# stdstu12/YUME

Measured on NVIDIA H100. Metric: latent_frames_per_sec, higher is better.
Workload: dtype bf16

## Files before the change

### yume_b200/build.py

```python
from __future__ import annotations

import hashlib
import os
import shutil
import subprocess
import sys
from pathlib import Path

ROOT = Path(__file__).resolve().parent
CSRC = ROOT / "csrc"
LIB = CSRC / "libyume_b200.so"
SOURCES = ["gemm.cu", "attention.cu", "elementwise.cu", "vae_elementwise.cu", "probe.cu", "clip.cu", "t5.cu", "gemm_fp8.cu",
           "attention_fp8.cu"]
HEADERS = ["yb_ptx.cuh", "yb_host.h", "../../include/yume_b200.h", "../../include/yume_b200_clip.h",
           "../../include/yume_b200_t5.h", "../../include/yume_b200_stream.h",
           "../../include/yume_b200_fp8.h", "../../include/yume_b200_fp8_attn.h",
           "../../include/yume_b200_fp8_vae.h"]

NVCC_FLAGS = [
    "-gencode", "arch=compute_90a,code=sm_90a",
    "-O3", "-lineinfo", "-std=c++17",
    "-Xcompiler", "-fPIC",
    "--expt-relaxed-constexpr",
    "-Xptxas", "-v",
# ... 19 lines not shown
    stamp = CSRC / ".build_stamp"
    digest = _digest()
    if not force and LIB.exists() and stamp.exists() and stamp.read_text().strip() == digest:
        return LIB
    nvcc = _nvcc()
    objs = []
    procs = []
    for src in SOURCES:
        obj = CSRC / (src[:-3] + ".o")
        cmd = [nvcc, *NVCC_FLAGS, "-c", str(CSRC / src), "-o", str(obj)]
        procs.append((src, obj, subprocess.Popen(cmd, stdout=subprocess.PIPE, stderr=subprocess.STDOUT, text=True)))
    log = []
    for src, obj, pr in procs:
        out, _ = pr.communicate()
        log.append(f"== {src}\n{out}")
        if pr.returncode != 0:
            sys.stderr.write("\n".join(log))
            raise RuntimeError(f"nvcc failed on {src}")
        objs.append(str(obj))
    tmp = LIB.with_suffix(".so.tmp")
    cmd = [nvcc, "-shared", "-gencode", "arch=compute_90a,code=sm_90a", "-o", str(tmp), *objs]
    r = subprocess.run(cmd, stdout=subprocess.PIPE, stderr=subprocess.STDOUT, text=True)
    if r.returncode != 0:
        sys.stderr.write(r.stdout)
        raise RuntimeError("nvcc link failed")
    os.replace(tmp, LIB)
    (CSRC / "build.log").write_text("\n".join(log))
    stamp.write_text(digest)
    if verbose:
        print("\n".join(log))
    return LIB


if __name__ == "__main__":
    p = build(force="--force" in sys.argv, verbose=True)
    print(f"built {p}")
```

### yume_b200/csrc/gemm.cu

```cuda
#include "yb_host.h"
#include "../../include/yume_b200_stream.h"
#include "yb_ptx.cuh"

namespace yb {

constexpr int GEMM_BLOCK_M = 128;
constexpr int GEMM_BLOCK_K = 64;
constexpr int GEMM_THREADS = 384;
constexpr int GEMM_MAX_STAGES = 8;
constexpr int GEMM_SMEM_BYTES = 227 * 1024;
constexpr int GEMM_A_BYTES = GEMM_BLOCK_M * GEMM_BLOCK_K * 2;
constexpr int GEMM_EPI_STAGE_BYTES = 8 * 16 * 36 * 4;
constexpr int GEMM_EPI_BOX_BYTES = 64 * 128;
constexpr int GEMM_EPI_TMA_BYTES = 2 * 2 * GEMM_EPI_BOX_BYTES;

struct GemmParams {
  int M, N, K;
  const float* bias;
  void* out;
  long long ldo;
  const float* gate;
  long long gate_ld;
  const int* tok_idx;
  int a_split;
  int n_split;
  long long split_stride;
  const __nv_bfloat16* res;
  long long res_ld;
  int conv, cin_chunks;
  int TW, TH, TT, tiles_w, tiles_h;
  int cT, cH, cW;
  int kh, kw;
  int off_t, off_h, off_w;
  int out_t_mul, out_t_add;
  int st_t, st_h, st_w;
  int num_m_tiles, num_n_tiles;
  int block_n, stages;
  int sk_full, sk_ns, sk_per;
  float* sk_ws;
  int tma_out;
  __nv_bfloat16* sp_peers[8];
  float* sp_sums;
  int sp_rank, sp_Lp, sp_Wh, sp_C;
};
constexpr int YB_EPI_SP_QKV = 6;

constexpr int CONVW_ROWS = GEMM_BLOCK_M + 2;
constexpr int CONVW_A_SLAB = 17 * 1024;
constexpr int CONVW_A_STAGES = 4;

__host__ __device__ constexpr int gemm_b_bytes(int block_n) { return ((block_n + 63) / 64) * 64 * GEMM_BLOCK_K * 2; }
__host__ __device__ constexpr int gemm_stage_bytes(int block_n, int convw) { return (convw ? 0 : GEMM_A_BYTES) + gemm_b_bytes(block_n); }
__host__ __device__ constexpr int gemm_a_ring_bytes(int convw) { return convw ? CONVW_A_STAGES * CONVW_A_SLAB : 0; }
__host__ __device__ constexpr bool gemm_has_tma_epilogue(int epi, int convw, int cluster) {
  return cluster == 1 && !convw && (epi == YB_EPI_BF16 || epi == YB_EPI_GELU_BF16 || epi == YB_EPI_GELU_ERF_BF16 ||
                                    epi == YB_EPI_F32 || epi == YB_EPI_GATE_RES);
}
__host__ __device__ constexpr bool gemm_tma_epilogue_only(int epi, int convw, int cluster) {
  return gemm_has_tma_epilogue(epi, convw, cluster) && epi != YB_EPI_BF16 && epi != YB_EPI_F32;
}
__host__ __device__ constexpr int gemm_epi_bytes(bool tma) { return tma ? GEMM_EPI_TMA_BYTES : GEMM_EPI_STAGE_BYTES; }
static int gemm_stages(int block_n, int convw, int epi_bytes) {
  const int s = (GEMM_SMEM_BYTES - 1024 - 256 - epi_bytes - gemm_a_ring_bytes(convw)) / gemm_stage_bytes(block_n, convw);
  return s > GEMM_MAX_STAGES ? GEMM_MAX_STAGES : s;
}

template <int EPI>
__device__ __forceinline__ void epilogue_rows16(const GemmParams& p, int col0, int my_row, int my_tok, const float* stage, int lane,
                                                float* sq) {
  constexpr bool kBf16Out = (EPI == YB_EPI_BF16 || EPI == YB_EPI_GELU_BF16 || EPI == YB_EPI_GELU_ERF_BF16 ||
                             EPI == YB_EPI_RES_BF16 || EPI == YB_EPI_SP_QKV);
  if (col0 >= p.N) return;
  if (kBf16Out) {
    const int cq = (lane & 3) * 8;
    float b[8] = {0.f, 0.f, 0.f, 0.f, 0.f, 0.f, 0.f, 0.f};
    if (p.bias) {
      const float4 b0 = __ldg(reinterpret_cast<const float4*>(p.bias + col0 + cq));
      const float4 b1 = __ldg(reinterpret_cast<const float4*>(p.bias + col0 + cq + 4));
      b[0] = b0.x; b[1] = b0.y; b[2] = b0.z; b[3] = b0.w; b[4] = b1.x; b[5] = b1.y; b[6] = b1.z; b[7] = b1.w;
    }
    long long col_off = col0 + cq;
    if (p.n_split > 0) col_off = static_cast<long long>(col0 / p.n_split) * p.split_stride + (col0 % p.n_split) + cq;
    __nv_bfloat16* obase = reinterpret_cast<__nv_bfloat16*>(p.out) + col_off;
    long long ld = p.ldo;
    if (EPI == YB_EPI_SP_QKV) {
      const int part = col0 / p.sp_C, cin = col0 - part * p.sp_C;
      const int peer = cin / p.sp_Wh;
      ld = 3LL * p.sp_Wh;
      obase = p.sp_peers[peer] + static_cast<long long>(p.sp_rank) * p.sp_Lp * ld + part * p.sp_Wh + (cin - peer * p.sp_Wh) + cq;
// ... 156 lines not shown
        if (EPI == YB_EPI_GATE_RES) tma_reduce_add_2d(tmO, buf, col0 + s * BOX_COLS, row0);
        else tma_store_2d(tmO, buf, col0 + s * BOX_COLS, row0);
        bulk_commit();
      }
      ++nbox;
    }
  }
}

template <int NM>
__device__ __forceinline__ void gemm_mma_k64(float (&acc)[128], uint32_t sa, uint32_t sb, int block_n, bool zero_first) {
  const uint64_t ad0 = make_smem_desc_sw128(sa, 16, 1024), bd0 = make_smem_desc_sw128(sb, 16, 1024);
  const int nb64 = (block_n + 63) >> 6;
#pragma unroll
  for (int k = 0; k < GEMM_BLOCK_K / 16; ++k) {
    const uint64_t ad = ad0 + 2 * k, bd = bd0 + 2 * k;
    const uint32_t accum = (zero_first && k == 0) ? 0u : 1u;
    if (NM == 256) {
      wgmma_ss_n256<0>(acc, ad, bd, accum);
    } else if (NM == 128) {
      wgmma_ss_n128<0>(acc, ad, bd, accum);
    } else {
      wgmma_ss_n64<0>(acc, ad, bd, accum);
      if (nb64 > 1) wgmma_ss_n64<32>(acc, ad, bd + (8192 >> 4), accum);
      if (nb64 > 2) wgmma_ss_n64<64>(acc, ad, bd + (16384 >> 4), accum);
      if (nb64 > 3) wgmma_ss_n64<96>(acc, ad, bd + (24576 >> 4), accum);
    }
  }
}

template <int CLUSTER>
__device__ __forceinline__ void release_slot(uint64_t* bar, int lane) {
  __syncwarp();
  if (lane == 0) {
    if (CLUSTER == 1) {
      mbar_arrive(bar);
    } else {
      mbar_arrive_cluster(bar, 0);
      mbar_arrive_cluster(bar, 1);
    }
  }
}

template <int EPI, int CONVW, int CLUSTER, int NM>
__global__ void __launch_bounds__(GEMM_THREADS, 1)
gemm_kernel(const __grid_constant__ CUtensorMap tmA, const __grid_constant__ CUtensorMap tmB, const __grid_constant__ CUtensorMap tmO,
            const GemmParams p) {
  static_assert(!(CONVW && CLUSTER != 1), "the kw-fused conv runs on single CTAs");
  constexpr bool kTmaEpi = gemm_has_tma_epilogue(EPI, CONVW, CLUSTER);
  const bool tma_out = gemm_tma_epilogue_only(EPI, CONVW, CLUSTER) || (kTmaEpi && p.tma_out);
  extern __shared__ uint8_t smem_raw[];
  uint8_t* smem = reinterpret_cast<uint8_t*>((reinterpret_cast<uintptr_t>(smem_raw) + 1023) & ~uintptr_t(1023));
  const int block_n = p.block_n, stages = p.stages;
  const int stage_bytes = gemm_stage_bytes(block_n, CONVW);
  uint8_t* a_ring = smem + stages * stage_bytes;
  float* epi = reinterpret_cast<float*>(a_ring + gemm_a_ring_bytes(CONVW));
  uint64_t* full_bar = reinterpret_cast<uint64_t*>(reinterpret_cast<uint8_t*>(epi) + gemm_epi_bytes(kTmaEpi));
  uint64_t* empty_bar = full_bar + GEMM_MAX_STAGES;
  uint64_t* a_full = empty_bar + GEMM_MAX_STAGES;
  uint64_t* a_empty = a_full + CONVW_A_STAGES;

  const int warp = threadIdx.x >> 5, lane = threadIdx.x & 31;
  const int rank = CLUSTER == 2 ? static_cast<int>(cluster_ctarank()) : 0;
  const int tile_first = blockIdx.x / CLUSTER, tile_step = gridDim.x / CLUSTER;
  const int num_tiles = p.num_m_tiles * p.num_n_tiles;
  const int num_kb = (p.K + GEMM_BLOCK_K - 1) / GEMM_BLOCK_K;
  const int num_work = p.sk_full + (num_tiles - p.sk_full) * p.sk_ns;
  auto decode_work = [&](int w, int& tile, int& kb0, int& kb1, int& part) {
    tile = w; kb0 = 0; kb1 = num_kb; part = -1;
    if (w >= p.sk_full) {
      const int u = w - p.sk_full;
      tile = p.sk_full + u / p.sk_ns;
      kb0 = (u % p.sk_ns) * p.sk_per;
      kb1 = min(num_kb, kb0 + p.sk_per);
      part = u;
    }
  };
  auto conv_box = [&](int mt, int& it, int& ih, int& iw) {
    const int per_t = p.tiles_h * p.tiles_w;
    it = mt / per_t;
    const int rem = mt - it * per_t;
    ih = rem / p.tiles_w;
    iw = rem - ih * p.tiles_w;
  };

  if (threadIdx.x == 0) {
    tma_prefetch_desc(&tmA);
    tma_prefetch_desc(&tmB);
    if (tma_out) tma_prefetch_desc(&tmO);
    for (int i = 0; i < stages; ++i) {
      mbar_init(&full_bar[i], 1);
      mbar_init(&empty_bar[i], 8 * CLUSTER);
    }
    for (int i = 0; i < (CONVW ? CONVW_A_STAGES : 0); ++i) {
      mbar_init(&a_full[i], 1);
      mbar_init(&a_empty[i], 8);
// ... 12 lines not shown
        int tile, kb0, kb1, part, m_tile, n_tile;
        decode_work(w, tile, kb0, kb1, part);
        tile_coords(tile, p.num_m_tiles, p.num_n_tiles, m_tile, n_tile);
        if (CONVW) {
          int it, ih, iw;
          conv_box(m_tile, it, ih, iw);
          const int groups = num_kb / 3;
          for (int g = 0; g < groups; ++g) {
            const int tdh = g / p.cin_chunks, cc = g - tdh * p.cin_chunks;
            const int dt = tdh / p.kh, dh = tdh - dt * p.kh;
            mbar_wait(&a_empty[a_stage], a_phase ^ 1);
            mbar_arrive_expect_tx(&a_full[a_stage], CONVW_ROWS * GEMM_BLOCK_K * 2);
            tma_load_4d(a_ring + a_stage * CONVW_A_SLAB, &tmA, &a_full[a_stage], cc * GEMM_BLOCK_K, iw * GEMM_BLOCK_M - p.off_w,
                        ih + dh - p.off_h, it + dt - p.off_t);
            if (++a_stage == CONVW_A_STAGES) {
              a_stage = 0;
              a_phase ^= 1;
            }
#pragma unroll 1
            for (int dw = 0; dw < 3; ++dw) {
              mbar_wait(&empty_bar[stage], phase ^ 1);
              mbar_arrive_expect_tx(&full_bar[stage], block_n * GEMM_BLOCK_K * 2);
              tma_load_2d(smem + stage * stage_bytes, &tmB, &full_bar[stage], ((tdh * 3 + dw) * p.cin_chunks + cc) * GEMM_BLOCK_K,
                          n_tile * block_n);
              if (++stage == stages) {
                stage = 0;
                phase ^= 1;
              }
            }
          }
          continue;
        }
        for (int kb = kb0; kb < kb1; ++kb) {
          if (CLUSTER > 1) mbar_wait_cluster(&empty_bar[stage], phase ^ 1);
          else mbar_wait(&empty_bar[stage], phase ^ 1);
          uint8_t* sa = smem + stage * stage_bytes;
          uint8_t* sb = sa + GEMM_A_BYTES;
          mbar_arrive_expect_tx(&full_bar[stage], GEMM_A_BYTES + block_n * GEMM_BLOCK_K * 2);
          const int kcol = kb * GEMM_BLOCK_K;
          const int mt = m_tile * CLUSTER + rank;
          if (p.conv) {
            const int tap = kb / p.cin_chunks, cc = kb - tap * p.cin_chunks;
            const int dt = tap / (p.kh * p.kw), dh = (tap / p.kw) % p.kh, dw = tap % p.kw;
            int it, ih, iw;
            conv_box(mt, it, ih, iw);
            tma_load_4d(sa, &tmA, &full_bar[stage], cc * GEMM_BLOCK_K, iw * p.TW * p.st_w + dw - p.off_w,
                        ih * p.TH * p.st_h + dh - p.off_h, it * p.TT * p.st_t + dt - p.off_t);
          } else {
            const int chunk = kcol / p.a_split;
            tma_load_3d(sa, &tmA, &full_bar[stage], kcol - chunk * p.a_split, mt * GEMM_BLOCK_M, chunk);
          }
          if (CLUSTER == 1) {
            tma_load_2d(sb, &tmB, &full_bar[stage], kcol, n_tile * block_n);
          } else {
            const int half = block_n / 2;
            tma_load_2d_multicast(sb + rank * half * GEMM_BLOCK_K * 2, &tmB, &full_bar[stage], kcol, n_tile * block_n + rank * half,
                                  static_cast<uint16_t>(3));
          }
          if (++stage == stages) {
            stage = 0;
            phase ^= 1;
          }
        }
      }
    }
  } else {
    setmaxnreg_inc<232>();
    const int wg = (warp >> 2) - 1;
// ... 40 lines not shown
          const uint32_t sa = smem_u32(a_ring + a_stage * CONVW_A_SLAB) + wg * 64 * 128;
#pragma unroll 1
          for (int dw = 0; dw < 3; ++dw) {
            mbar_wait(&full_bar[stage], phase);
            fence_regs(acc);
            wgmma_fence();
            gemm_mma_k64<NM>(acc, sa + dw * 128, smem_u32(smem + stage * stage_bytes), block_n, g == 0 && dw == 0);
            wgmma_commit();
            wgmma_wait<1>();
            fence_regs(acc);
            if (prev >= 0) release_slot<1>(&empty_bar[prev], lane);
            if (dw == 0 && prev_a >= 0) {
              release_slot<1>(&a_empty[prev_a], lane);
              prev_a = -1;
            }
            prev = stage;
            if (++stage == stages) {
              stage = 0;
              phase ^= 1;
            }
          }
          prev_a = a_stage;
          if (++a_stage == CONVW_A_STAGES) {
            a_stage = 0;
            a_phase ^= 1;
          }
        }
        wgmma_wait<0>();
        fence_regs(acc);
        if (prev >= 0) release_slot<1>(&empty_bar[prev], lane);
        if (prev_a >= 0) release_slot<1>(&a_empty[prev_a], lane);
      } else {
        for (int kb = kb0; kb < kb1; ++kb) {
          mbar_wait(&full_bar[stage], phase);
          const uint32_t sa = smem_u32(smem + stage * stage_bytes);
          fence_regs(acc);
          wgmma_fence();
          gemm_mma_k64<NM>(acc, sa + wg * 64 * 128, sa + GEMM_A_BYTES, block_n, kb == kb0);
          wgmma_commit();
          wgmma_wait<1>();
          fence_regs(acc);
          if (prev >= 0) release_slot<CLUSTER>(&empty_bar[prev], lane);
          prev = stage;
          if (++stage == stages) {
            stage = 0;
            phase ^= 1;
          }
        }
        wgmma_wait<0>();
        fence_regs(acc);
        if (prev >= 0) release_slot<CLUSTER>(&empty_bar[prev], lane);
      }

      const int q4 = lane >> 2, c2 = 2 * (lane & 3);
      if (part >= 0) {
        float* wbase = p.sk_ws + (static_cast<long long>(part) * 256 + rank * GEMM_BLOCK_M + r0) * block_n;
#pragma unroll
        for (int g = 0; g < 32; ++g) {
          if (g * 8 < block_n) {
            *reinterpret_cast<float2*>(wbase + q4 * block_n + g * 8 + c2) = make_float2(acc[4 * g], acc[4 * g + 1]);
            *reinterpret_cast<float2*>(wbase + (q4 + 8) * block_n + g * 8 + c2) = make_float2(acc[4 * g + 2], acc[4 * g + 3]);
          }
        }
        continue;
      }
      if (tma_out) {
        epilogue_tma<EPI, NM>(p, &tmO, acc, box_bufs, mt * GEMM_BLOCK_M + wg * 64, n_tile * block_n, wg, threadIdx.x & 127, nbox);
        continue;
      }
      int my_tok = 0;
      if (EPI == YB_EPI_GATE_RES && p.gate != nullptr && p.tok_idx != nullptr && my_row >= 0) my_tok = p.tok_idx[my_row];
      float sq[2] = {0.f, 0.f};
      auto flush_sq = [&](int part_) {
#pragma unroll
        for (int it = 0; it < 2; ++it) {
          float v = sq[it];
          v += __shfl_xor_sync(0xffffffffu, v, 1);
          v += __shfl_xor_sync(0xffffffffu, v, 2);
          const int rowi = __shfl_sync(0xffffffffu, my_row, it * 8 + (lane >> 2));
          if ((lane & 3) == 0 && rowi >= 0 && part_ < 2) atomicAdd(p.sp_sums + rowi * 2 + part_, v);
          sq[it] = 0.f;
        }
      };
      int cur_part = (EPI == YB_EPI_SP_QKV) ? (n_tile * block_n) / p.sp_C : 0;
#pragma unroll
      for (int c = 0; c < 8; ++c) {
        if (c * 32 < block_n) {
#pragma unroll
          for (int g = 0; g < 4; ++g) {
            const int i = 4 * (4 * c + g);
            *reinterpret_cast<float2*>(stage_buf + q4 * 36 + g * 8 + c2) = make_float2(acc[i], acc[i + 1]);
            *reinterpret_cast<float2*>(stage_buf + (q4 + 8) * 36 + g * 8 + c2) = make_float2(acc[i + 2], acc[i + 3]);
          }
          __syncwarp();
          const int col0 = n_tile * block_n + c * 32;
          if (EPI == YB_EPI_SP_QKV && col0 < p.N) {
            const int pt = col0 / p.sp_C;
            if (pt != cur_part) {
              flush_sq(cur_part);
              cur_part = pt;
            }
          }
          epilogue_rows16<EPI>(p, col0, my_row, my_tok, stage_buf, lane, sq);
          __syncwarp();
        }
      }
      if (EPI == YB_EPI_SP_QKV) flush_sq(cur_part);
    }
    if (tma_out && (threadIdx.x & 127) == 0) bulk_wait<0>();
  }
  if (CLUSTER > 1) cluster_sync_all();
}

__global__ void __launch_bounds__(256) gemm_splitk_combine_kernel(const GemmParams p, int tail_tiles) {
  const int block_n = p.block_n, quads = block_n >> 2;
  const long long total = static_cast<long long>(tail_tiles) * 256 * quads;
  for (long long i = blockIdx.x * static_cast<long long>(blockDim.x) + threadIdx.x; i < total;
       i += static_cast<long long>(gridDim.x) * blockDim.x) {
    const int cq = static_cast<int>(i % quads) * 4;
    const long long rr = i / quads;
    const int r = static_cast<int>(rr & 255);
    const int t = static_cast<int>(rr >> 8);
    int m_tile, n_tile;
    tile_coords(p.sk_full + t, p.num_m_tiles, p.num_n_tiles, m_tile, n_tile);
    const int row = m_tile * 256 + r, col = n_tile * block_n + cq;
    if (row >= p.M || col >= p.N) continue;
    float4 a = make_float4(0.f, 0.f, 0.f, 0.f);
    for (int sg = 0; sg < p.sk_ns; ++sg) {
      const float4 v = *reinterpret_cast<const float4*>(p.sk_ws + ((static_cast<long long>(t) * p.sk_ns + sg) * 256 + r) * block_n + cq);
      a.x += v.x; a.y += v.y; a.z += v.z; a.w += v.w;
    }
    if (p.bias) {
      const float4 b = __ldg(reinterpret_cast<const float4*>(p.bias + col));
      a.x += b.x; a.y += b.y; a.z += b.z; a.w += b.w;
    }
    float4 g = make_float4(1.f, 1.f, 1.f, 1.f);
    if (p.gate) {
      const long long tok = p.tok_idx ? p.tok_idx[row] : 0;
      g = __ldg(reinterpret_cast<const float4*>(p.gate + tok * p.gate_ld + col));
    }
    float4* xp = reinterpret_cast<float4*>(reinterpret_cast<float*>(p.out) + static_cast<long long>(row) * p.ldo + col);
    float4 x = *xp;
    x.x += a.x * g.x; x.y += a.y * g.y; x.z += a.z * g.z; x.w += a.w * g.w;
// ... 26 lines not shown
}

static int pair_block_n(int M, int N, int clusters) {
  (void)M;
  (void)clusters;
  return N >= 256 ? 256 : ((N + 31) / 32) * 32;
}

template <typename Kern>
static int pair_max_clusters(Kern kern) {
  cudaLaunchConfig_t cfg = {};
  cfg.gridDim = dim3(2 * (sm_count() / 2));
  cfg.blockDim = dim3(GEMM_THREADS);
  cfg.dynamicSmemBytes = GEMM_SMEM_BYTES;
  cudaLaunchAttribute attr;
  attr.id = cudaLaunchAttributeClusterDimension;
  attr.val.clusterDim.x = 2;
  attr.val.clusterDim.y = 1;
  attr.val.clusterDim.z = 1;
  cfg.attrs = &attr;
  cfg.numAttrs = 1;
  int n = 0;
  if (cudaOccupancyMaxActiveClusters(&n, kern, &cfg) != cudaSuccess || n <= 0) {
    (void)cudaGetLastError();
    n = sm_count() / 2;
  }
  return n;
}

template <int EPI, int CONVW, int CLUSTER>
static int launch_gemm(const CUtensorMap& tmA, const CUtensorMap& tmB, const CUtensorMap* tmO, GemmParams& p, cudaStream_t stream,
                       int split_k = 1, void* ws = nullptr, long long ws_bytes = 0) {
  static const CUtensorMap no_map = {};
  if (gemm_tma_epilogue_only(EPI, CONVW, CLUSTER) && tmO == nullptr) return YB_ERR_ARG;
  p.tma_out = gemm_has_tma_epilogue(EPI, CONVW, CLUSTER) && tmO != nullptr;
  if (!p.tma_out) tmO = &no_map;
  const int nm = p.block_n == 256 ? 2 : p.block_n == 128 ? 1 : 0;
  if (CLUSTER == 1 && nm == 0) return YB_ERR_ARG;
  auto kern = nm == 2 ? gemm_kernel<EPI, CONVW, CLUSTER, 256> : nm == 1 ? gemm_kernel<EPI, CONVW, CLUSTER, 128>
                      : gemm_kernel<EPI, CONVW, CLUSTER, CLUSTER == 1 ? 128 : 64>;
  static bool attr_set[3][kMaxDevices] = {};
  if (int rc = ensure_dynamic_smem(kern, GEMM_SMEM_BYTES, attr_set[nm], "gemm")) return rc;
  if (CLUSTER == 2) p.num_m_tiles = p.conv ? (p.num_m_tiles + 1) / 2 : (p.M + 255) / 256;
  else if (!p.conv) p.num_m_tiles = (p.M + GEMM_BLOCK_M - 1) / GEMM_BLOCK_M;
  p.num_n_tiles = (p.N + p.block_n - 1) / p.block_n;
  p.stages = gemm_stages(p.block_n, CONVW, gemm_epi_bytes(gemm_has_tma_epilogue(EPI, CONVW, CLUSTER)));
  const int tiles = p.num_m_tiles * p.num_n_tiles;
  static int max_clusters[kMaxDevices] = {0};
  const int dev = current_device();
  if (max_clusters[dev] == 0) max_clusters[dev] = CLUSTER == 2 ? pair_max_clusters(kern) : sm_count();
  p.sk_full = tiles; p.sk_ns = 1; p.sk_per = 0; p.sk_ws = nullptr;
  int tail = 0;
  if (CLUSTER == 2 && EPI == YB_EPI_GATE_RES && !p.conv && ws != nullptr && split_k != 1) {
    const int num_kb = (p.K + GEMM_BLOCK_K - 1) / GEMM_BLOCK_K;
    gemm_splitk_plan(tiles, num_kb, max_clusters[dev], split_k, &p.sk_full, &p.sk_ns, &p.sk_per);
    tail = tiles - p.sk_full;
    const long long need = static_cast<long long>(tail) * p.sk_ns * 256 * p.block_n * 4;
    if (tail > 0 && (ws_bytes < need || (reinterpret_cast<uintptr_t>(ws) & 0xF))) {
      p.sk_full = tiles; p.sk_ns = 1; tail = 0;
    }
    if (tail > 0) p.sk_ws = static_cast<float*>(ws);
  }
  const int work = p.sk_full + tail * p.sk_ns;
  const int groups = work < max_clusters[dev] ? work : max_clusters[dev];
  cudaLaunchConfig_t cfg = {};
  cfg.gridDim = dim3(groups * CLUSTER);
  cfg.blockDim = dim3(GEMM_THREADS);
  cfg.dynamicSmemBytes = GEMM_SMEM_BYTES;
  cfg.stream = stream;
  cudaLaunchAttribute attr;
  attr.id = cudaLaunchAttributeClusterDimension;
  attr.val.clusterDim.x = CLUSTER;
  attr.val.clusterDim.y = 1;
  attr.val.clusterDim.z = 1;
  cfg.attrs = &attr;
  cfg.numAttrs = 1;
  (void)cudaLaunchKernelEx(&cfg, kern, tmA, tmB, *tmO, p);
  int rc = check_launch("gemm");
  if (rc || tail == 0) return rc;
// ... 107 lines not shown
  if (a->struct_bytes != sizeof(yb_gemm_args)) return YB_ERR_ARG;
  if (a->cta_pair < 0 || a->cta_pair > 2 || a->split_k < 0 || a->split_k > 12) return YB_ERR_ARG;
  int a_split = a->K;
  long long a_chunk_ld = 0;
  if (a->a_split > 0) {
    if (a->a_split % GEMM_BLOCK_K != 0 || a->K % a->a_split != 0) return YB_ERR_SHAPE;
    a_split = a->a_split;
    a_chunk_ld = a->a_split_stride;
  }
  const int a_chunks = a->K / a_split;
  if (a->n_split < 0 || (a->n_split > 0 && (a->n_split % 32 != 0 || a->epilogue != YB_EPI_BF16))) return YB_ERR_ARG;
  GemmParams p;
  p.M = a->M;
  p.N = a->N;
  p.K = a->K;
  p.bias = static_cast<const float*>(a->bias);
  p.out = a->out;
  p.ldo = a->ldo;
  p.gate = static_cast<const float*>(a->gate);
  p.gate_ld = a->gate_ld;
  p.tok_idx = static_cast<const int*>(a->tok_idx);
  p.a_split = a_split;
  p.res = static_cast<const __nv_bfloat16*>(a->res);
  p.res_ld = a->res_ld;
  p.conv = 0;
  p.n_split = a->n_split;
  p.split_stride = a->split_stride;
  p.block_n = 0;
  p.stages = 0;
  CUtensorMap tmA, tmB;
  int rc = make_tmap_bf16_3d(&tmA, a->A, a_chunks, a->M, a_split, a->lda, a_chunks > 1 ? a_chunk_ld : a->lda * (long long)a->M + 8,
                             GEMM_BLOCK_M, GEMM_BLOCK_K);
  if (rc) return rc;
  const bool pair = a->cta_pair == 2;
  if (pair) {
    int bn = a->block_n;
    if (bn == 0) bn = pair_block_n(a->M, a->N, sm_count() / 2);
    if (bn < 32 || bn > 256 || bn % 32 != 0) return YB_ERR_ARG;
    p.block_n = bn;
    rc = make_tmap_bf16_2d(&tmB, a->B, a->N, a->K, a->ldb, bn / 2, GEMM_BLOCK_K);
    if (rc) return rc;
    switch (a->epilogue) {
      case YB_EPI_BF16: return launch_gemm<YB_EPI_BF16, 0, 2>(tmA, tmB, nullptr, p, stream);
      case YB_EPI_GELU_BF16: return launch_gemm<YB_EPI_GELU_BF16, 0, 2>(tmA, tmB, nullptr, p, stream);
      case YB_EPI_F32: return launch_gemm<YB_EPI_F32, 0, 2>(tmA, tmB, nullptr, p, stream);
      case YB_EPI_GELU_ERF_BF16: return launch_gemm<YB_EPI_GELU_ERF_BF16, 0, 2>(tmA, tmB, nullptr, p, stream);
      case YB_EPI_RES_BF16: return launch_gemm<YB_EPI_RES_BF16, 0, 2>(tmA, tmB, nullptr, p, stream);
      default: return launch_gemm<YB_EPI_GATE_RES, 0, 2>(tmA, tmB, nullptr, p, stream, a->split_k, a->ws, a->ws_bytes);
    }
  }
  const int block_n = (a->block_n == 128 || a->block_n == 256) ? a->block_n : ((a->N % 256 == 0 || a->N > 1024) ? 256 : 128);
  rc = make_tmap_bf16_2d(&tmB, a->B, a->N, a->K, a->ldb, block_n, GEMM_BLOCK_K);
  if (rc) return rc;
  p.block_n = block_n;
  CUtensorMap tmO;
  const CUtensorMap* tmo = nullptr;
  if (a->n_split == 0 && a->epilogue != YB_EPI_RES_BF16) {
    const int elem = (a->epilogue == YB_EPI_F32 || a->epilogue == YB_EPI_GATE_RES) ? 4 : 2;
    rc = make_tmap_out_2d(&tmO, a->out, a->M, a->N, a->ldo, elem, 64);
    if (rc) return rc;
    tmo = &tmO;
  }
  switch (a->epilogue) {
    case YB_EPI_BF16: return launch_gemm<YB_EPI_BF16, 0, 1>(tmA, tmB, tmo, p, stream);
    case YB_EPI_GELU_BF16: return launch_gemm<YB_EPI_GELU_BF16, 0, 1>(tmA, tmB, tmo, p, stream);
    case YB_EPI_F32: return launch_gemm<YB_EPI_F32, 0, 1>(tmA, tmB, tmo, p, stream);
    case YB_EPI_GELU_ERF_BF16: return launch_gemm<YB_EPI_GELU_ERF_BF16, 0, 1>(tmA, tmB, tmo, p, stream);
    case YB_EPI_RES_BF16: return launch_gemm<YB_EPI_RES_BF16, 0, 1>(tmA, tmB, nullptr, p, stream);
    default: return launch_gemm<YB_EPI_GATE_RES, 0, 1>(tmA, tmB, tmo, p, stream);
  }
}


static int conv3d_launch(const yb_conv3d_args* a, int t_hist, void* stream_) {
  using namespace yb;
  if (!a || !a->xpad || !a->w || !a->out) return YB_ERR_ARG;
  if (a->struct_bytes != sizeof(yb_conv3d_args)) return YB_ERR_ARG;
  if (a->T <= 0 || a->H <= 0 || a->W <= 0 || a->Cp <= 0 || a->Cout <= 0) return YB_ERR_ARG;
  if (t_hist < 0) return YB_ERR_ARG;
  if (a->Cp % 64 != 0 || a->Cout % 32 != 0) return YB_ERR_SHAPE;
  if ((a->ldo % 8) || (reinterpret_cast<uintptr_t>(a->out) & 0xF)) return YB_ERR_ALIGNMENT;
  if (a->epilogue != YB_EPI_BF16 && a->epilogue != YB_EPI_F32 && a->epilogue != YB_EPI_RES_BF16) return YB_ERR_ARG;
  if (a->epilogue == YB_EPI_RES_BF16 && (!a->res || (a->res_ld % 8))) return YB_ERR_ARG;
  cudaStream_t stream = reinterpret_cast<cudaStream_t>(stream_);
  GemmParams p;
  const int kt = a->kt > 0 ? a->kt : 3, kh = a->kh > 0 ? a->kh : 3, kw = a->kw > 0 ? a->kw : 3;
  if ((kt != 1 && kt != 3) || (kh != 1 && kh != 3) || (kw != 1 && kw != 3)) return YB_ERR_SHAPE;
  const int block_n = (a->Cout % 256 == 0) ? 256 : 128;
  bool fuse_w = false;
  if (a->cta_pair < 0 || a->cta_pair > 2) return YB_ERR_ARG;
  const int st_t = a->stride_t > 0 ? a->stride_t : 1, st_hw = a->stride_hw > 0 ? a->stride_hw : 1;
  if (st_t > 2 || st_hw > 2) return YB_ERR_ARG;
  const bool strided = st_t > 1 || st_hw > 1;
  if (strided && !a->oob_zero_pad) return YB_ERR_ARG;
  if (t_hist > 0 && (!a->oob_zero_pad || t_hist != (st_t > 1 ? 1 : kt - 1))) return YB_ERR_ARG;
// ... 41 lines not shown
    p.conv = 1;
    p.block_n = a->Cout <= 256 ? a->Cout : (a->Cout % 192 == 0 ? 192 : 256);
    CUtensorMap tmBp;
    rc = make_tmap_bf16_2d(&tmBp, a->w, a->Cout, static_cast<uint64_t>(taps) * a->Cp, static_cast<uint64_t>(taps) * a->Cp,
                           p.block_n / 2, GEMM_BLOCK_K);
    if (rc) return rc;
    switch (a->epilogue) {
      case YB_EPI_BF16: return launch_gemm<YB_EPI_BF16, 0, 2>(tmA, tmBp, nullptr, p, stream);
      case YB_EPI_F32: return launch_gemm<YB_EPI_F32, 0, 2>(tmA, tmBp, nullptr, p, stream);
      default: return launch_gemm<YB_EPI_RES_BF16, 0, 2>(tmA, tmBp, nullptr, p, stream);
    }
  }
  p.block_n = block_n;
#define YB_CONV_DISPATCH(CW)                                                                  \
  switch (a->epilogue) {                                                                     \
    case YB_EPI_BF16: return launch_gemm<YB_EPI_BF16, CW, 1>(tmA, tmB, nullptr, p, stream);   \
    case YB_EPI_F32: return launch_gemm<YB_EPI_F32, CW, 1>(tmA, tmB, nullptr, p, stream);     \
    default: return launch_gemm<YB_EPI_RES_BF16, CW, 1>(tmA, tmB, nullptr, p, stream);        \
  }
  if (fuse_w) {
    YB_CONV_DISPATCH(1)
  } else {
    YB_CONV_DISPATCH(0)
  }
#undef YB_CONV_DISPATCH
}

extern "C" int yb_conv3d_causal(const yb_conv3d_args* a, void* stream) { return conv3d_launch(a, 0, stream); }

extern "C" int yb_conv3d_causal_hist(const yb_conv3d_args* a, int t_hist, void* stream) {
  if (t_hist <= 0) return YB_ERR_ARG;
  return conv3d_launch(a, t_hist, stream);
}
```

### yume_b200/csrc/yb_ptx.cuh

```cuda
#pragma once
#include <cstdint>
#include <cstdio>
#include <cuda.h>
#include <cuda_runtime.h>
#include <cuda_bf16.h>

namespace yb {

__device__ __forceinline__ uint32_t smem_u32(const void* p) {
  return static_cast<uint32_t>(__cvta_generic_to_shared(p));
}

template <int N>
__device__ __forceinline__ void setmaxnreg_inc() {
  asm volatile("setmaxnreg.inc.sync.aligned.u32 %0;\n" ::"n"(N));
}
template <int N>
__device__ __forceinline__ void setmaxnreg_dec() {
  asm volatile("setmaxnreg.dec.sync.aligned.u32 %0;\n" ::"n"(N));
}
__device__ __forceinline__ void named_bar_sync(int id, int count) {
  asm volatile("bar.sync %0, %1;" ::"r"(id), "r"(count) : "memory");
}

// ... 35 lines not shown
      : "memory");
  return ok != 0;
}
#ifndef YB_WAIT_LIMIT_CYCLES
#define YB_WAIT_LIMIT_CYCLES 8000000000LL
#endif
__device__ __forceinline__ void mbar_wait(uint64_t* bar, uint32_t parity) {
  if (mbar_try_wait(bar, parity)) return;
  const long long t0 = clock64();
  while (!mbar_try_wait(bar, parity)) {
    if (clock64() - t0 > YB_WAIT_LIMIT_CYCLES) {
#ifdef YB_DEBUG_WAIT
      printf("yb: mbarrier wait timeout block=(%d,%d) thread=%d bar=%u parity=%u\n", blockIdx.x, blockIdx.y,
             threadIdx.x, smem_u32(bar), parity);
#endif
      __trap();
    }
  }
}
__device__ __forceinline__ void att_wait(uint64_t* bar, uint32_t parity) {
  if (mbar_try_wait(bar, parity)) return;
  const long long t0 = clock64();
  while (!mbar_try_wait(bar, parity)) {
    if (clock64() - t0 > YB_WAIT_LIMIT_CYCLES) {
#ifdef YB_DEBUG_WAIT
      printf("yb: attention consumer mbarrier wait timeout block=(%d,%d) thread=%d bar=%u parity=%u\n", blockIdx.x,
             blockIdx.y, threadIdx.x, smem_u32(bar), parity);
#endif
      asm volatile("trap;");
      break;
    }
  }
}
__device__ __forceinline__ void mbar_wait_cluster(uint64_t* bar, uint32_t parity) {
  const long long t0 = clock64();
  for (;;) {
    uint32_t ok;
    asm volatile(
        "{\n\t.reg .pred p;\n\t"
        "mbarrier.try_wait.parity.acquire.cluster.shared::cta.b64 p, [%1], %2;\n\t"
        "selp.u32 %0, 1, 0, p;\n\t}\n"
        : "=r"(ok)
        : "r"(smem_u32(bar)), "r"(parity)
        : "memory");
    if (ok) return;
    if (clock64() - t0 > YB_WAIT_LIMIT_CYCLES) __trap();
  }
}

__device__ __forceinline__ uint32_t cluster_ctarank() {
  uint32_t r;
  asm volatile("mov.u32 %0, %%cluster_ctarank;" : "=r"(r));
  return r;
}
__device__ __forceinline__ void cluster_sync_all() {
  asm volatile("barrier.cluster.arrive.release.aligned;\n\tbarrier.cluster.wait.acquire.aligned;" ::: "memory");
}
__device__ __forceinline__ void mbar_arrive_cluster(uint64_t* bar, uint32_t cta) {
  uint32_t remote;
  asm volatile("mapa.shared::cluster.u32 %0, %1, %2;" : "=r"(remote) : "r"(smem_u32(bar)), "r"(cta));
  asm volatile("mbarrier.arrive.release.cluster.shared::cluster.b64 _, [%0];" ::"r"(remote) : "memory");
}

__device__ __forceinline__ void tma_prefetch_desc(const CUtensorMap* tmap) {
  asm volatile("prefetch.tensormap [%0];" ::"l"(reinterpret_cast<uint64_t>(tmap)) : "memory");
}
__device__ __forceinline__ void tma_load_2d(void* smem_dst, const CUtensorMap* tmap, uint64_t* bar, int c0, int c1) {
  asm volatile(
      "cp.async.bulk.tensor.2d.shared::cluster.global.tile.mbarrier::complete_tx::bytes [%0], [%1, {%3, %4}], [%2];"
      ::"r"(smem_u32(smem_dst)), "l"(reinterpret_cast<uint64_t>(tmap)), "r"(smem_u32(bar)), "r"(c0), "r"(c1)
      : "memory");
}
__device__ __forceinline__ void tma_load_2d_multicast(void* smem_dst, const CUtensorMap* tmap, uint64_t* bar, int c0, int c1,
                                                      uint16_t mask) {
  asm volatile(
      "cp.async.bulk.tensor.2d.shared::cluster.global.mbarrier::complete_tx::bytes.multicast::cluster [%0], [%1, {%3, %4}], "
      "[%2], %5;" ::"r"(smem_u32(smem_dst)),
      "l"(reinterpret_cast<uint64_t>(tmap)), "r"(smem_u32(bar)), "r"(c0), "r"(c1), "h"(mask)
      : "memory");
}
__device__ __forceinline__ void tma_load_3d(void* smem_dst, const CUtensorMap* tmap, uint64_t* bar, int c0, int c1,
                                            int c2) {
  asm volatile(
      "cp.async.bulk.tensor.3d.shared::cluster.global.tile.mbarrier::complete_tx::bytes [%0], [%1, {%3, %4, %5}], [%2];"
      ::"r"(smem_u32(smem_dst)), "l"(reinterpret_cast<uint64_t>(tmap)), "r"(smem_u32(bar)), "r"(c0), "r"(c1), "r"(c2)
      : "memory");
}
__device__ __forceinline__ void tma_load_4d(void* smem_dst, const CUtensorMap* tmap, uint64_t* bar, int c0, int c1,
                                            int c2, int c3) {
  asm volatile(
      "cp.async.bulk.tensor.4d.shared::cluster.global.tile.mbarrier::complete_tx::bytes [%0], [%1, {%3, %4, %5, %6}], [%2];"
      ::"r"(smem_u32(smem_dst)), "l"(reinterpret_cast<uint64_t>(tmap)), "r"(smem_u32(bar)), "r"(c0), "r"(c1), "r"(c2),
      "r"(c3)
      : "memory");
// ... 136 lines not shown
```

Measured before the change: 41.45.

## Enable TMA store epilogue for CTA-pair GEMMs and relax cluster barrier semantics

Extends the TMA-based output epilogue to the two-CTA cluster GEMM path, building the output tensor map before the pair branch and passing it in, except for the 64-wide N template. It also drops the cluster-acquire wait and cluster-release arrive in favour of plain mbarrier ops, and has two lanes send the two remote arrivals in parallel. Optional profiling counters, a no-MMA probe mode and a variant-build helper are added behind defines. Removing the release/acquire ordering on cross-CTA empty barriers could allow a producer to overwrite a slot before the peer's reads are visible.

```diff
diff --git a/yume_b200/build.py b/yume_b200/build.py
--- a/yume_b200/build.py
+++ b/yume_b200/build.py
@@ -75,6 +75,28 @@
     return LIB
 
 
+def build_variant(define: str, out_dir: Path) -> Path:
+    build()
+    out_dir = Path(out_dir)
+    out_dir.mkdir(parents=True, exist_ok=True)
+    nvcc = _nvcc()
+    obj = out_dir / "gemm.o"
+    r = subprocess.run([nvcc, *NVCC_FLAGS, f"-D{define}", "-c", str(CSRC / "gemm.cu"), "-o", str(obj)],
+                       stdout=subprocess.PIPE, stderr=subprocess.STDOUT, text=True)
+    (out_dir / "build.log").write_text(r.stdout)
+    if r.returncode != 0:
+        sys.stderr.write(r.stdout)
+        raise RuntimeError(f"nvcc failed on gemm.cu -D{define}")
+    objs = [str(obj)] + [str(CSRC / (s[:-3] + ".o")) for s in SOURCES if s != "gemm.cu"]
+    lib = out_dir / LIB.name
+    r = subprocess.run([nvcc, "-shared", "-gencode", "arch=compute_90a,code=sm_90a", "-o", str(lib), *objs],
+                       stdout=subprocess.PIPE, stderr=subprocess.STDOUT, text=True)
+    if r.returncode != 0:
+        sys.stderr.write(r.stdout)
+        raise RuntimeError("nvcc link failed")
+    return lib
+
+
 if __name__ == "__main__":
     p = build(force="--force" in sys.argv, verbose=True)
     print(f"built {p}")
diff --git a/yume_b200/csrc/gemm.cu b/yume_b200/csrc/gemm.cu
--- a/yume_b200/csrc/gemm.cu
+++ b/yume_b200/csrc/gemm.cu
@@ -13,6 +13,14 @@
 constexpr int GEMM_EPI_STAGE_BYTES = 8 * 16 * 36 * 4;
 constexpr int GEMM_EPI_BOX_BYTES = 64 * 128;
 constexpr int GEMM_EPI_TMA_BYTES = 2 * 2 * GEMM_EPI_BOX_BYTES;
+
+#ifdef YB_GEMM_PROFILE
+constexpr int GEMM_PROF_CTAS = 1024, GEMM_PROF_FIELDS = 8;
+__device__ long long g_gemm_prof[GEMM_PROF_CTAS][GEMM_PROF_FIELDS];
+#define YB_GEMM_TIMED(sum, stmt) do { const long long t0_ = clock64(); stmt; (sum) += clock64() - t0_; } while (0)
+#else
+#define YB_GEMM_TIMED(sum, stmt) do { stmt; } while (0)
+#endif
 
 struct GemmParams {
   int M, N, K;
@@ -53,8 +61,8 @@
 __host__ __device__ constexpr int gemm_stage_bytes(int block_n, int convw) { return (convw ? 0 : GEMM_A_BYTES) + gemm_b_bytes(block_n); }
 __host__ __device__ constexpr int gemm_a_ring_bytes(int convw) { return convw ? CONVW_A_STAGES * CONVW_A_SLAB : 0; }
 __host__ __device__ constexpr bool gemm_has_tma_epilogue(int epi, int convw, int cluster) {
-  return cluster == 1 && !convw && (epi == YB_EPI_BF16 || epi == YB_EPI_GELU_BF16 || epi == YB_EPI_GELU_ERF_BF16 ||
-                                    epi == YB_EPI_F32 || epi == YB_EPI_GATE_RES);
+  return !convw && (epi == YB_EPI_BF16 || epi == YB_EPI_GELU_BF16 || epi == YB_EPI_GELU_ERF_BF16 || epi == YB_EPI_F32 ||
+                    epi == YB_EPI_GATE_RES);
 }
 __host__ __device__ constexpr bool gemm_tma_epilogue_only(int epi, int convw, int cluster) {
   return gemm_has_tma_epilogue(epi, convw, cluster) && epi != YB_EPI_BF16 && epi != YB_EPI_F32;
@@ -277,13 +285,10 @@
 template <int CLUSTER>
 __device__ __forceinline__ void release_slot(uint64_t* bar, int lane) {
   __syncwarp();
-  if (lane == 0) {
-    if (CLUSTER == 1) {
-      mbar_arrive(bar);
-    } else {
-      mbar_arrive_cluster(bar, 0);
-      mbar_arrive_cluster(bar, 1);
-    }
+  if (CLUSTER == 1) {
+    if (lane == 0) mbar_arrive(bar);
+  } else if (lane < 2) {
+    mbar_arrive_cluster(bar, lane);
   }
 }
 
@@ -292,8 +297,8 @@
 gemm_kernel(const __grid_constant__ CUtensorMap tmA, const __grid_constant__ CUtensorMap tmB, const __grid_constant__ CUtensorMap tmO,
             const GemmParams p) {
   static_assert(!(CONVW && CLUSTER != 1), "the kw-fused conv runs on single CTAs");
-  constexpr bool kTmaEpi = gemm_has_tma_epilogue(EPI, CONVW, CLUSTER);
-  const bool tma_out = gemm_tma_epilogue_only(EPI, CONVW, CLUSTER) || (kTmaEpi && p.tma_out);
+  constexpr bool kTmaEpi = gemm_has_tma_epilogue(EPI, CONVW, CLUSTER) && NM != 64;
+  const bool tma_out = kTmaEpi && (gemm_tma_epilogue_only(EPI, CONVW, CLUSTER) || p.tma_out);
   extern __shared__ uint8_t smem_raw[];
   uint8_t* smem = reinterpret_cast<uint8_t*>((reinterpret_cast<uintptr_t>(smem_raw) + 1023) & ~uintptr_t(1023));
   const int block_n = p.block_n, stages = p.stages;
@@ -307,6 +312,10 @@
 
   const int warp = threadIdx.x >> 5, lane = threadIdx.x & 31;
   const int rank = CLUSTER == 2 ? static_cast<int>(cluster_ctarank()) : 0;
+#ifdef YB_GEMM_PROFILE
+  const long long prof_t0 = clock64();
+  long long prof_empty = 0, prof_full = 0, prof_release = 0, prof_epi = 0, prof_items = 0;
+#endif
   const int tile_first = blockIdx.x / CLUSTER, tile_step = gridDim.x / CLUSTER;
   const int num_tiles = p.num_m_tiles * p.num_n_tiles;
   const int num_kb = (p.K + GEMM_BLOCK_K - 1) / GEMM_BLOCK_K;
@@ -385,8 +394,7 @@
           continue;
         }
         for (int kb = kb0; kb < kb1; ++kb) {
-          if (CLUSTER > 1) mbar_wait_cluster(&empty_bar[stage], phase ^ 1);
-          else mbar_wait(&empty_bar[stage], phase ^ 1);
+          YB_GEMM_TIMED(prof_empty, mbar_wait(&empty_bar[stage], phase ^ 1));
           uint8_t* sa = smem + stage * stage_bytes;
           uint8_t* sb = sa + GEMM_A_BYTES;
           mbar_arrive_expect_tx(&full_bar[stage], GEMM_A_BYTES + block_n * GEMM_BLOCK_K * 2);
@@ -493,7 +501,10 @@
         if (prev_a >= 0) release_slot<1>(&a_empty[prev_a], lane);
       } else {
         for (int kb = kb0; kb < kb1; ++kb) {
-          mbar_wait(&full_bar[stage], phase);
+          YB_GEMM_TIMED(prof_full, mbar_wait(&full_bar[stage], phase));
+#ifdef YB_GEMM_NO_MMA
+          YB_GEMM_TIMED(prof_release, release_slot<CLUSTER>(&empty_bar[stage], lane));
+#else
           const uint32_t sa = smem_u32(smem + stage * stage_bytes);
           fence_regs(acc);
           wgmma_fence();
@@ -501,8 +512,9 @@
           wgmma_commit();
           wgmma_wait<1>();
           fence_regs(acc);
-          if (prev >= 0) release_slot<CLUSTER>(&empty_bar[prev], lane);
+          if (prev >= 0) YB_GEMM_TIMED(prof_release, release_slot<CLUSTER>(&empty_bar[prev], lane));
           prev = stage;
+#endif
           if (++stage == stages) {
             stage = 0;
             phase ^= 1;
@@ -525,8 +537,15 @@
         }
         continue;
       }
+#ifdef YB_GEMM_PROFILE
+      ++prof_items;
+      const long long prof_e0 = clock64();
+#endif
       if (tma_out) {
         epilogue_tma<EPI, NM>(p, &tmO, acc, box_bufs, mt * GEMM_BLOCK_M + wg * 64, n_tile * block_n, wg, threadIdx.x & 127, nbox);
+#ifdef YB_GEMM_PROFILE
+        prof_epi += clock64() - prof_e0;
+#endif
         continue;
       }
       int my_tok = 0;
@@ -567,9 +586,31 @@
         }
       }
       if (EPI == YB_EPI_SP_QKV) flush_sq(cur_part);
+#ifdef YB_GEMM_PROFILE
+      prof_epi += clock64() - prof_e0;
+#endif
     }
     if (tma_out && (threadIdx.x & 127) == 0) bulk_wait<0>();
   }
+#ifdef YB_GEMM_PROFILE
+  if (blockIdx.x < GEMM_PROF_CTAS) {
+    long long* row = g_gemm_prof[blockIdx.x];
+    if (threadIdx.x == 0) {
+      row[0] = prof_empty;
+      row[4] = clock64() - prof_t0;
+      uint32_t smid;
+      asm volatile("mov.u32 %0, %%smid;" : "=r"(smid));
+      row[6] = smid;
+      row[7] = gridDim.x;
+    }
+    if (threadIdx.x == 128) {
+      row[1] = prof_full;
+      row[2] = prof_release;
+      row[3] = prof_epi;
+      row[5] = prof_items;
+    }
+  }
+#endif
   if (CLUSTER > 1) cluster_sync_all();
 }
 
@@ -662,11 +703,12 @@
 static int launch_gemm(const CUtensorMap& tmA, const CUtensorMap& tmB, const CUtensorMap* tmO, GemmParams& p, cudaStream_t stream,
                        int split_k = 1, void* ws = nullptr, long long ws_bytes = 0) {
   static const CUtensorMap no_map = {};
-  if (gemm_tma_epilogue_only(EPI, CONVW, CLUSTER) && tmO == nullptr) return YB_ERR_ARG;
-  p.tma_out = gemm_has_tma_epilogue(EPI, CONVW, CLUSTER) && tmO != nullptr;
-  if (!p.tma_out) tmO = &no_map;
   const int nm = p.block_n == 256 ? 2 : p.block_n == 128 ? 1 : 0;
   if (CLUSTER == 1 && nm == 0) return YB_ERR_ARG;
+  const bool has_tma = gemm_has_tma_epilogue(EPI, CONVW, CLUSTER) && nm != 0;
+  if (has_tma && gemm_tma_epilogue_only(EPI, CONVW, CLUSTER) && tmO == nullptr) return YB_ERR_ARG;
+  p.tma_out = has_tma && tmO != nullptr;
+  if (!p.tma_out) tmO = &no_map;
   auto kern = nm == 2 ? gemm_kernel<EPI, CONVW, CLUSTER, 256> : nm == 1 ? gemm_kernel<EPI, CONVW, CLUSTER, 128>
                       : gemm_kernel<EPI, CONVW, CLUSTER, CLUSTER == 1 ? 128 : 64>;
   static bool attr_set[3][kMaxDevices] = {};
@@ -674,7 +716,7 @@
   if (CLUSTER == 2) p.num_m_tiles = p.conv ? (p.num_m_tiles + 1) / 2 : (p.M + 255) / 256;
   else if (!p.conv) p.num_m_tiles = (p.M + GEMM_BLOCK_M - 1) / GEMM_BLOCK_M;
   p.num_n_tiles = (p.N + p.block_n - 1) / p.block_n;
-  p.stages = gemm_stages(p.block_n, CONVW, gemm_epi_bytes(gemm_has_tma_epilogue(EPI, CONVW, CLUSTER)));
+  p.stages = gemm_stages(p.block_n, CONVW, gemm_epi_bytes(has_tma));
   const int tiles = p.num_m_tiles * p.num_n_tiles;
   static int max_clusters[kMaxDevices] = {0};
   const int dev = current_device();
@@ -848,8 +890,15 @@
   int rc = make_tmap_bf16_3d(&tmA, a->A, a_chunks, a->M, a_split, a->lda, a_chunks > 1 ? a_chunk_ld : a->lda * (long long)a->M + 8,
                              GEMM_BLOCK_M, GEMM_BLOCK_K);
   if (rc) return rc;
-  const bool pair = a->cta_pair == 2;
-  if (pair) {
+  CUtensorMap tmO;
+  const CUtensorMap* tmo = nullptr;
+  if (a->n_split == 0 && a->epilogue != YB_EPI_RES_BF16) {
+    const int elem = (a->epilogue == YB_EPI_F32 || a->epilogue == YB_EPI_GATE_RES) ? 4 : 2;
+    rc = make_tmap_out_2d(&tmO, a->out, a->M, a->N, a->ldo, elem, 64);
+    if (rc) return rc;
+    tmo = &tmO;
+  }
+  if (a->cta_pair == 2) {
     int bn = a->block_n;
     if (bn == 0) bn = pair_block_n(a->M, a->N, sm_count() / 2);
     if (bn < 32 || bn > 256 || bn % 32 != 0) return YB_ERR_ARG;
@@ -857,26 +906,18 @@
     rc = make_tmap_bf16_2d(&tmB, a->B, a->N, a->K, a->ldb, bn / 2, GEMM_BLOCK_K);
     if (rc) return rc;
     switch (a->epilogue) {
-      case YB_EPI_BF16: return launch_gemm<YB_EPI_BF16, 0, 2>(tmA, tmB, nullptr, p, stream);
-      case YB_EPI_GELU_BF16: return launch_gemm<YB_EPI_GELU_BF16, 0, 2>(tmA, tmB, nullptr, p, stream);
-      case YB_EPI_F32: return launch_gemm<YB_EPI_F32, 0, 2>(tmA, tmB, nullptr, p, stream);
-      case YB_EPI_GELU_ERF_BF16: return launch_gemm<YB_EPI_GELU_ERF_BF16, 0, 2>(tmA, tmB, nullptr, p, stream);
+      case YB_EPI_BF16: return launch_gemm<YB_EPI_BF16, 0, 2>(tmA, tmB, tmo, p, stream);
+      case YB_EPI_GELU_BF16: return launch_gemm<YB_EPI_GELU_BF16, 0, 2>(tmA, tmB, tmo, p, stream);
+      case YB_EPI_F32: return launch_gemm<YB_EPI_F32, 0, 2>(tmA, tmB, tmo, p, stream);
+      case YB_EPI_GELU_ERF_BF16: return launch_gemm<YB_EPI_GELU_ERF_BF16, 0, 2>(tmA, tmB, tmo, p, stream);
       case YB_EPI_RES_BF16: return launch_gemm<YB_EPI_RES_BF16, 0, 2>(tmA, tmB, nullptr, p, stream);
-      default: return launch_gemm<YB_EPI_GATE_RES, 0, 2>(tmA, tmB, nullptr, p, stream, a->split_k, a->ws, a->ws_bytes);
+      default: return launch_gemm<YB_EPI_GATE_RES, 0, 2>(tmA, tmB, tmo, p, stream, a->split_k, a->ws, a->ws_bytes);
     }
   }
   const int block_n = (a->block_n == 128 || a->block_n == 256) ? a->block_n : ((a->N % 256 == 0 || a->N > 1024) ? 256 : 128);
   rc = make_tmap_bf16_2d(&tmB, a->B, a->N, a->K, a->ldb, block_n, GEMM_BLOCK_K);
   if (rc) return rc;
   p.block_n = block_n;
-  CUtensorMap tmO;
-  const CUtensorMap* tmo = nullptr;
-  if (a->n_split == 0 && a->epilogue != YB_EPI_RES_BF16) {
-    const int elem = (a->epilogue == YB_EPI_F32 || a->epilogue == YB_EPI_GATE_RES) ? 4 : 2;
-    rc = make_tmap_out_2d(&tmO, a->out, a->M, a->N, a->ldo, elem, 64);
-    if (rc) return rc;
-    tmo = &tmO;
-  }
   switch (a->epilogue) {
     case YB_EPI_BF16: return launch_gemm<YB_EPI_BF16, 0, 1>(tmA, tmB, tmo, p, stream);
     case YB_EPI_GELU_BF16: return launch_gemm<YB_EPI_GELU_BF16, 0, 1>(tmA, tmB, tmo, p, stream);
@@ -984,3 +1025,15 @@
   if (t_hist <= 0) return YB_ERR_ARG;
   return conv3d_launch(a, t_hist, stream);
 }
+
+#ifdef YB_GEMM_PROFILE
+extern "C" int yb_gemm_prof_read(long long* out, int max_ctas) {
+  using namespace yb;
+  if (!out || max_ctas <= 0) return YB_ERR_ARG;
+  const int n = max_ctas < GEMM_PROF_CTAS ? max_ctas : GEMM_PROF_CTAS;
+  if (cudaMemcpyFromSymbol(out, g_gemm_prof, sizeof(long long) * GEMM_PROF_FIELDS * n) != cudaSuccess) return YB_ERR_LAUNCH;
+  static long long zeros[GEMM_PROF_CTAS][GEMM_PROF_FIELDS] = {};
+  if (cudaMemcpyToSymbol(g_gemm_prof, zeros, sizeof(zeros)) != cudaSuccess) return YB_ERR_LAUNCH;
+  return YB_OK;
+}
+#endif
diff --git a/yume_b200/csrc/yb_ptx.cuh b/yume_b200/csrc/yb_ptx.cuh
--- a/yume_b200/csrc/yb_ptx.cuh
+++ b/yume_b200/csrc/yb_ptx.cuh
@@ -91,21 +91,6 @@
     }
   }
 }
-__device__ __forceinline__ void mbar_wait_cluster(uint64_t* bar, uint32_t parity) {
-  const long long t0 = clock64();
-  for (;;) {
-    uint32_t ok;
-    asm volatile(
-        "{\n\t.reg .pred p;\n\t"
-        "mbarrier.try_wait.parity.acquire.cluster.shared::cta.b64 p, [%1], %2;\n\t"
-        "selp.u32 %0, 1, 0, p;\n\t}\n"
-        : "=r"(ok)
-        : "r"(smem_u32(bar)), "r"(parity)
-        : "memory");
-    if (ok) return;
-    if (clock64() - t0 > YB_WAIT_LIMIT_CYCLES) __trap();
-  }
-}
 
 __device__ __forceinline__ uint32_t cluster_ctarank() {
   uint32_t r;
@@ -118,7 +103,7 @@
 __device__ __forceinline__ void mbar_arrive_cluster(uint64_t* bar, uint32_t cta) {
   uint32_t remote;
   asm volatile("mapa.shared::cluster.u32 %0, %1, %2;" : "=r"(remote) : "r"(smem_u32(bar)), "r"(cta));
-  asm volatile("mbarrier.arrive.release.cluster.shared::cluster.b64 _, [%0];" ::"r"(remote) : "memory");
+  asm volatile("mbarrier.arrive.shared::cluster.b64 _, [%0];" ::"r"(remote) : "memory");
 }
 
 __device__ __forceinline__ void tma_prefetch_desc(const CUtensorMap* tmap) {
```

After: 41.48, median of 6. Within noise of the previous version (+0.1%).
